# vitoplantamura/OnnxStream

Hardware: NVIDIA H100
Metric: SD1.5 UNet 512x512 bs=1 denoise steps/s (one UNet Model::run per step) (higher is better)
Workload: dtype f16

## Files before the change

### include/onnxstream_b200_kernels.h

```cpp
#ifndef ONNXSTREAM_B200_KERNELS_H
#define ONNXSTREAM_B200_KERNELS_H

#include <stddef.h>
#include <stdint.h>

#ifdef __cplusplus
extern "C" {
#endif

enum { OSB_NONE = 0, OSB_U8 = 1, OSB_F16 = 2, OSB_F32 = 3, OSB_I64 = 4 };

#define OSB_MAX_DIMS 6

int osb_convert(const void* src, int src_dtype, void* dst, int dst_dtype, size_t n, float scale, int zero_point, void* stream);

enum { OSB_UN_SIGMOID = 0, OSB_UN_SILU, OSB_UN_ERF, OSB_UN_SQRT, OSB_UN_SIN, OSB_UN_COS, OSB_UN_POW, OSB_UN_NEG,
       OSB_UN_GELU_ERF, OSB_UN_COPY, OSB_UN_MULC, OSB_UN_ADDC, OSB_UN_RECIP_SQRT };
int osb_unary(int op, const void* x, void* y, int dtype, size_t n, float alpha, void* stream);

enum { OSB_BIN_ADD = 0, OSB_BIN_SUB, OSB_BIN_MUL, OSB_BIN_DIV, OSB_BIN_MUL_GELU, OSB_BIN_MUL_SIGMOID, OSB_BIN_SILU_MUL  };
int osb_binary(int op, const void* a, const int64_t* a_strides, const void* b, const int64_t* b_strides,
               void* out, const int64_t* out_shape, int ndim, int dtype, void* stream);

int osb_bf16x3_expand_cols(const void* in_f32, void* out_bf16, int64_t rows, int64_t L, int64_t ld_in, int b_side, void* stream);
// ... 7 lines not shown
int osb_tc_gemm_f32x_f16w(const void* A_f32, const void* B_f16, int64_t ldb, void* C_f32, const void* bias_f32, const void* residual_f32, int64_t M, int64_t N,
                          int64_t K, void* planes, void* stream);
int osb_tc_conv_f32x_f16w_ok(int64_t H, int64_t W, int64_t Cin, int64_t Cout, int kh, int kw, int stride, int64_t Ho, int64_t Wo);
int osb_tc_conv_f32x_f16w(const void* x_f32, const void* w_f16, const void* bias_f32, const void* residual_f32, void* y_f32, int64_t H, int64_t W, int64_t Cin,
                          int64_t Cout, int kh, int kw, int stride, int pad_top, int pad_left, int64_t Ho, int64_t Wo, void* planes, void* stream);
int osb_concat2(const void* a, const void* b, void* out, int64_t outer, int64_t a_bytes, int64_t b_bytes, void* stream);
int osb_strided_copy(const void* in, void* out, int elem_size, int ndim, const int64_t* shape,
                     const int64_t* in_stride, const int64_t* in_div, int64_t in_offset,
                     const int64_t* out_stride, int64_t out_offset, void* stream);

int osb_transpose2d(const void* in, void* out, int elem_size, int64_t batch, int64_t rows, int64_t cols, void* stream);

int osb_softmax(const void* x, void* y, int dtype, int64_t rows, int64_t cols, void* stream);

int osb_softmax_scaled(const void* x, void* y, int dtype, int64_t rows, int64_t cols, float scale, const void* mask, int64_t mask_rows, void* stream);
int osb_softmax_scaled_ld(const void* x, void* y, int dtype, int64_t rows, int64_t cols, int64_t ld, float scale, const void* mask, int64_t mask_rows, void* stream);

int osb_instance_norm(const void* x, void* y, int dtype, int64_t channels, int64_t n_per_channel,
                      const void* scale, const void* bias, float eps, void* stream);

int osb_group_norm(const void* x, void* y, int dtype, int nhwc, int64_t C, int64_t HW, int groups,
                   const void* gamma, const void* beta, float eps, int fuse_silu, void* stats, void* stream);

int osb_geglu(const void* x, void* y, int dtype, int64_t rows, int64_t inner, void* stream);
int osb_tc_gemm_geglu(const void* A, const void* B, void* y, const void* bias, int64_t M, int64_t inner, int64_t K, void* stream);

int osb_layer_norm(const void* x, void* y, int dtype, int64_t rows, int64_t cols, const void* gamma, const void* beta,
                   float eps, void* stream);

int osb_reduce_mean(const void* x, void* y, int dtype, int64_t rows, int64_t cols, void* stream);

int osb_gather_rows(const void* table, const int64_t* idx, void* out, int64_t n_idx, int64_t table_rows, int64_t row_bytes, void* stream);

int osb_gemm(const void* A, const void* B, void* C, const void* bias, const void* residual,
             int64_t batch, int64_t M, int64_t N, int64_t K,
             int64_t stride_a, int64_t stride_b, int64_t stride_c, int b_transposed, int dtype, int impl, void* stream);

int osb_gemm_grouped(const void* A, const void* const* B, void* const* C, int groups, int64_t M, int64_t N, int64_t K,
                     int b_transposed, int dtype, int impl, void* stream);

int osb_gemm_ld(const void* A, int64_t lda, const void* B, int64_t ldb, void* C, int64_t ldc, const void* bias, const void* residual,
                int64_t batch, int64_t M, int64_t N, int64_t K, int64_t stride_a, int64_t stride_b, int64_t stride_c,
                int b_transposed, int dtype, int impl, void* stream);

int osb_conv2d(const void* x, const void* w, const void* bias, const void* residual, void* y,
               int64_t H, int64_t W, int64_t Cin, int64_t Cout, int kh, int kw, int stride, int pad_top, int pad_left,
               int64_t Ho, int64_t Wo, int dtype, int impl, void* stream);
int osb_conv2d_ex(const void* x, const void* w, const void* bias, const void* bias2, const void* residual, void* y, int64_t H, int64_t W, int64_t Cin, int64_t Cout,
                  int kh, int kw, int stride, int pad_top, int pad_left, int64_t Ho, int64_t Wo, int dtype, int impl, void* stream,
                  void* gn_stats, int gn_groups, int* gn_done);
int osb_conv2d_fusable(const void* x, const void* w, const void* y, int64_t H, int64_t W, int64_t Cin, int64_t Cout, int kh, int kw, int stride, int dtype, int impl);
int osb_rms_norm(const void* x, int xd, const void* w, int wd, void* y, int yd, int64_t rows, int64_t cols, float eps, void* stream);
int osb_rope(const void* x, const void* cs, const void* sn, void* y, int dtype, int64_t rows, int64_t D, int64_t table_rows, void* stream);
int osb_gemv_w8(const void* A, const void* Wq, void* C, const void* bias, const void* residual, int64_t M, int64_t N, int64_t K, float wscale, int wzp, int dtype, void* stream);
int osb_gemv_f16w(const void* A, const void* W, int64_t ldb, void* C, const void* bias, const void* residual, int64_t M, int64_t N, int64_t K, void* stream);
int osb_gemv_grouped(const void* A, const void* const* B, void* const* C, const int64_t* N, const float* wscale, const int* wzp, int groups,
                     int64_t M, int64_t K, int wdtype, int dtype, void* stream);
int osb_qu8_tc_gemm_ok(int64_t M, int64_t N, int64_t K, const void* A, const void* B, const void* C);
int osb_qu8_tc_conv_ok(int64_t Cin, int64_t Cout, int64_t Ho, int64_t Wo, int kh, int kw, int stride, const void* x, const void* w, const void* y);
int osb_rowsum_u8(const void* x, void* out, int64_t rows, int64_t cols, void* stream);
int osb_colsum_u8(const void* w, void* out, int64_t K, int64_t N, void* stream);
int osb_pad_sum_u8(const void* x, void* xp, void* psum, int64_t H, int64_t W, int64_t C, int64_t Hp, int64_t Wp, int pad_top, int pad_left, int zx, void* stream);
int osb_qu8_tc_gemm(const void* A, const void* B, void* C, const void* bias, const void* rsum, const void* csum, int64_t M, int64_t N, int64_t K, int bt,
                    int zx, float sx, int zw, float sw, int zy, float sy, void* stream);
int osb_qu8_tc_conv(const void* xp, const void* psum, const void* w, const void* bias, const void* csum, void* y, int64_t Hp, int64_t Wp, int64_t Cin, int64_t Cout,
                    int kh, int kw, int stride, int64_t Ho, int64_t Wo, int zx, float sx, int zw, float sw, int zy, float sy, void* stream);
int osb_binary_qu8(int op, const void* a, const int64_t* as, float sa, int za, const void* b, const int64_t* bs, float sb, int zb,
                   void* out, float so, int zo, const int64_t* shape, int ndim, void* stream);
int osb_softmax_qu8(const void* x, void* y, int64_t rows, int64_t cols, float in_scale, float out_scale, int out_zp, void* stream);
int osb_percentiles(const void* x, int dtype, size_t n, int threads, float from_left, float from_right, void* out3, void* stream);
float osb_percentile_key_to_float(unsigned key, int dtype);
int osb_channel_add_stats(const void* x, const void* addv, void* y, int dtype, int64_t C, int64_t HW, int groups, void* stats, void* stream);
int osb_concat2_stats(const void* a, const void* b, void* y, int dtype, int64_t ca, int64_t cb, int64_t HW, int groups, void* stats, void* stream);
int osb_group_norm_apply(const void* x, void* y, int dtype, int64_t C, int64_t HW, int groups, const void* gamma, const void* beta, float eps, int fuse_silu,
                         const void* stats, void* clear_stats, void* stream);

int osb_attention(const void* q, const void* k, const void* v, const void* mask, void* out,
                  int64_t heads, int64_t Tq, int64_t Tk, int64_t d, int64_t dv, float scale, int k_transposed,
                  int64_t kv_group, int dtype, void* stream);

int osb_flash_attention_ok(int64_t T, int64_t Tk, int64_t d, int dtype);
int osb_flash_attention(const void* q, int64_t ldq, const void* k, int64_t ldk, const void* v, int64_t ldv, void* out, int64_t ldo,
                        int64_t heads, int64_t T, int64_t Tk, int64_t d, float scale, void* stream);

int osb_flash_attention_f32x_ok(int64_t T, int64_t Tk, int64_t d, int dtype);
int osb_flash_attention_f32x(const void* q, int64_t ldq, const void* k, int64_t ldk, const void* v, int64_t ldv, void* out, int64_t ldo,
                             int64_t heads, int64_t T, int64_t Tk, int64_t d, float scale, void* planes, void* stream);

int osb_flash_attention_wide_ok(int64_t T, int64_t Tk, int64_t d, int dtype);
int osb_flash_attention_wide(const void* q, const void* k, const void* v, void* out, int64_t heads, int64_t T, int64_t Tk, int64_t d,
                             float scale, int k_transposed, int dtype, void* stream);

int osb_flash_attention_wide_f32x_ok(int64_t T, int64_t Tk, int64_t d, int dtype);
int osb_flash_attention_wide_f32x(const void* q, const void* k, const void* v, void* out, int64_t heads, int64_t T, int64_t Tk, int64_t d,
                                  float scale, int k_transposed, void* planes, void* stream);

int osb_sdpa_flash_ok(int64_t Hq, int64_t Hkv, int64_t Tq, int64_t Tk, int64_t d, int64_t dv, int dtype);
int osb_sdpa_flash(const void* q, const void* k, const void* v, const void* mask, void* out,
                   int64_t Hq, int64_t Hkv, int64_t Tq, int64_t Tk, int64_t d, float scale, void* stream);

int osb_sdpa_flash_f32x_ok(int64_t Hq, int64_t Hkv, int64_t Tq, int64_t Tk, int64_t d, int64_t dv, int dtype);
int osb_sdpa_flash_f32x(const void* q, const void* k, const void* v, const void* mask, void* out,
                        int64_t Hq, int64_t Hkv, int64_t Tq, int64_t Tk, int64_t d, float scale,
                        void* planes, void* stream);

int osb_gemm_qu8(const uint8_t* A, const uint8_t* B, uint8_t* C, const int32_t* bias, int64_t M, int64_t N, int64_t K,
                 int zx, float sx, int zw, float sw, int zy, float sy, void* stream);
int osb_conv2d_qu8(const uint8_t* x, const uint8_t* w, const int32_t* bias, uint8_t* y,
                   int64_t H, int64_t W, int64_t Cin, int64_t Cout, int kh, int kw, int stride, int pad_top, int pad_left,
                   int64_t Ho, int64_t Wo, int zx, float sx, int zw, float sw, int zy, float sy, void* stream);

int osb_scatter_elems(void* out, const int64_t* pos, const void* updates, int64_t n, int elem_size, void* stream);

int osb_maxpool_nhwc(const void* x, void* y, int dtype, int64_t H, int64_t W, int64_t C, int kh, int kw, int stride, int pad_top,
                     int pad_left, int64_t Ho, int64_t Wo, void* stream);

int osb_fill(void* dst, int dtype, size_t n, float value, void* stream);

int osb_gemm_tc_eligible(int64_t M, int64_t N, int64_t K, int dtype);

void osb_tc_set_pair_mode(int mode);

void osb_tc_set_tile(int bm, int bn, int split);

void osb_tc_profile(int enable);
int osb_tc_profile_read(double* out4);
int osb_tc_profile_dump(char* buf, int cap);

int osb_pdl_enabled(void);
void osb_set_pdl(int enable);

uint64_t osb_launch_count(void);
void osb_launch_count_reset(void);
uint64_t osb_tc_launch_count(void);

#ifdef __cplusplus
}
#endif
#endif
```

### onnxstream_b200/csrc/attention_wgmma.cu

```cuda

#include "common.cuh"
#include "tc_ptx.cuh"
#include <cuda.h>
#include <cstdio>

namespace {

using namespace tcptx;

constexpr int BQ = 128;
constexpr int BKV = 128;
constexpr int KV_STAGES = 4;
constexpr int FA_THREADS = 384;
constexpr int FA_CONSUMERS = 256;
constexpr int FA_PRODUCER_REGS = 40, FA_CONSUMER_REGS = 232;

template <int NCH, int BK, int QKS, int KS = KV_STAGES, int PLANES = 1>
struct FaCfg {
    static_assert(QKS <= 4 * NCH && (BK == 32 || BK == 64 || BK == 128), "tile");
    static constexpr int Q_CHUNK = BQ * 128;
    static constexpr int KV_CHUNK = BK * 128;
    static constexpr int Q_PLANE = NCH * Q_CHUNK;
    static constexpr int KV_PLANE = NCH * KV_CHUNK;
    static constexpr int Q_BYTES = PLANES * Q_PLANE;
    static constexpr int KV_BYTES = PLANES * KV_PLANE;
    static constexpr int BARS = Q_BYTES + KS * 2 * KV_BYTES;
    static constexpr int SMEM = BARS + 1024 + 256;
};

struct FaParams {
    int T, Tk, d;
    int kv_tiles;
    float scale_log2;
    __half* out;
    long long ldo;
};

__device__ __forceinline__ uint8_t* fa_prologue(const CUtensorMap* map_q, const CUtensorMap* map_k, const CUtensorMap* map_v, int bar_off,
                                                uint32_t arrivals, int n0, int n1 = 0)
{
    extern __shared__ uint8_t smem_raw[];
    uint8_t* smem = (uint8_t*)(((uintptr_t)smem_raw + 1023) & ~(uintptr_t)1023);
    const int warp = threadIdx.x >> 5, lane = threadIdx.x & 31;
    if (warp == 0 && lane == 0) {
        asm volatile("prefetch.tensormap [%0];" ::"l"(map_q) : "memory");
        asm volatile("prefetch.tensormap [%0];" ::"l"(map_k) : "memory");
        asm volatile("prefetch.tensormap [%0];" ::"l"(map_v) : "memory");
    }
    if (warp == 1 && lane == 0) {
        uint64_t* bars = (uint64_t*)(smem + bar_off);
        mbar_init(bars, 1);
        for (int i = 0; i < n0; i++) { mbar_init(&bars[1 + i], 1); mbar_init(&bars[1 + n0 + i], arrivals); }
        for (int i = 0; i < n1; i++) { mbar_init(&bars[1 + 2 * n0 + i], 1); mbar_init(&bars[1 + 2 * n0 + n1 + i], arrivals); }
        asm volatile("fence.mbarrier_init.release.cluster;" ::: "memory");
    }
    __syncthreads();
    osb_pdl_wait();
    return smem;
}

template <int KS, typename Load>
__device__ __forceinline__ void fa_produce_kv(uint64_t* kv_full, uint64_t* kv_empty, int n_kv, uint32_t tile_bytes, Load load)
{
    for (int j = 0; j < n_kv; j++) {
        const int st = j % KS;
        mbar_wait(&kv_empty[st], ((j / KS) & 1) ^ 1);
        if (elect_one()) {
            mbar_expect_tx(&kv_full[st], tile_bytes);
            load(st, j, &kv_full[st]);
        }
        __syncwarp();
    }
    osb_pdl_trigger_late();
}

template <int BK>
__device__ __forceinline__ float fa_row_max(const float (&s)[BK / 2], int h)
{
    float mt = -INFINITY;
#pragma unroll
    for (int c = 0; c < BK / 8; c++) mt = fmaxf(mt, fmaxf(s[4 * c + 2 * h], s[4 * c + 2 * h + 1]));
    mt = fmaxf(mt, __shfl_xor_sync(0xffffffffu, mt, 1));
    mt = fmaxf(mt, __shfl_xor_sync(0xffffffffu, mt, 2));
    return mt;
}

__device__ __forceinline__ float ex2_approx(float x)
{
    float y;
    asm("ex2.approx.ftz.f32 %0, %1;" : "=f"(y) : "f"(x));
    return y;
}

__device__ __forceinline__ uint32_t pack_half2(float lo, float hi)
{
    __half2 h2 = __floats2half2_rn(lo, hi);
    return *reinterpret_cast<uint32_t*>(&h2);
}

__device__ __forceinline__ void store_pair(__half* p, float lo, float hi) { *reinterpret_cast<uint32_t*>(p) = pack_half2(lo, hi); }
__device__ __forceinline__ void store_pair(float* p, float lo, float hi) { *reinterpret_cast<float2*>(p) = make_float2(lo, hi); }

template <typename OutT, int NCH>
__device__ __forceinline__ void fa_store(const float (&o)[NCH][32], const float (&l_run)[2], OutT* const (&rows)[2], int ncols, int cq)
{
#pragma unroll
    for (int h = 0; h < 2; h++) {
        float l = l_run[h];
        l += __shfl_xor_sync(0xffffffffu, l, 1);
        l += __shfl_xor_sync(0xffffffffu, l, 2);
        const float inv = 1.f / l;
        if (!rows[h]) continue;
#pragma unroll
        for (int ch = 0; ch < NCH; ch++)
#pragma unroll
            for (int c = 0; c < 8; c++) {
                const int col = 64 * ch + 8 * c + cq;
                if (col < ncols) store_pair(rows[h] + col, o[ch][4 * c + 2 * h] * inv, o[ch][4 * c + 2 * h + 1] * inv);
            }
    }
}

template <int BK>
__device__ __forceinline__ void qk_mma(float (&s)[BK / 2], uint64_t da, uint64_t db, uint32_t scale_d = 1u)
{
    if constexpr (BK == 128) wgmma_m64n128k16_f16<0>(s, da, db, scale_d);
    else if constexpr (BK == 64) wgmma_m64n64k16_f16<0>(s, da, db, scale_d);
    else wgmma_m64n32k16_f16<0>(s, da, db, scale_d);
}

template <int NCH, int BK, int QKS>
__device__ __forceinline__ void fa_issue_qk(float (&s)[BK / 2], uint64_t qdesc, uint64_t kdesc)
{
    using C = FaCfg<NCH, BK, QKS>;
    fence_regs(s);
    wgmma_fence();
#pragma unroll
    for (int k = 0; k < QKS; k++)
        qk_mma<BK>(s, qdesc + (uint64_t)(((k >> 2) * C::Q_CHUNK >> 4) + (k & 3) * 2), kdesc + (uint64_t)(((k >> 2) * C::KV_CHUNK >> 4) + (k & 3) * 2), k > 0);
    wgmma_commit();
}

template <int NCH, int BK, int QKS>
__device__ __forceinline__ void fa_issue_pv(float (&o)[NCH][32], uint32_t (&a)[BK / 16][4], uint64_t vdesc)
{
    using C = FaCfg<NCH, BK, QKS>;
#pragma unroll
    for (int ch = 0; ch < NCH; ch++) fence_regs(o[ch]);
    fence_regs(a);
    wgmma_fence();
#pragma unroll
    for (int kk = 0; kk < BK / 16; kk++)
#pragma unroll
        for (int ch = 0; ch < NCH; ch++)
            wgmma_m64n64k16_f16_rs(o[ch], a[kk], vdesc + (uint64_t)((ch * C::KV_CHUNK + kk * 2048) >> 4), 1u);
    wgmma_commit();
}

template <int BK>
__device__ __forceinline__ void fa_softmax(float (&s)[BK / 2], float (&m_run)[2], float (&l_run)[2], float (&alpha)[2], int key0, int cq, const FaParams& p)
{
    if (key0 + BK > p.Tk) {
#pragma unroll
        for (int c = 0; c < BK / 8; c++)
#pragma unroll
            for (int e = 0; e < 2; e++)
                if (key0 + 8 * c + cq + e >= p.Tk) { s[4 * c + e] = -INFINITY; s[4 * c + 2 + e] = -INFINITY; }
    }
    float neg_m[2];
#pragma unroll
    for (int h = 0; h < 2; h++) {
        const float m_new = fmaxf(m_run[h], fa_row_max<BK>(s, h) * p.scale_log2);
        alpha[h] = ex2_approx(m_run[h] - m_new);
        neg_m[h] = -m_new;
        m_run[h] = m_new;
    }
    float lsum[2] = { 0.f, 0.f };
#pragma unroll
    for (int c = 0; c < BK / 8; c++)
#pragma unroll
        for (int h = 0; h < 2; h++)
#pragma unroll
            for (int e = 0; e < 2; e++) {
                const float pe = ex2_approx(fmaf(s[4 * c + 2 * h + e], p.scale_log2, neg_m[h]));
                s[4 * c + 2 * h + e] = pe;
                lsum[h] += pe;
            }
#pragma unroll
    for (int h = 0; h < 2; h++) l_run[h] = l_run[h] * alpha[h] + lsum[h];
}

template <int NCH, int BK>
__device__ __forceinline__ void fa_rescale_pack(float (&o)[NCH][32], uint32_t (&a)[BK / 16][4], const float (&s)[BK / 2], const float (&alpha)[2])
{
#pragma unroll
    for (int ch = 0; ch < NCH; ch++)
#pragma unroll
        for (int c = 0; c < 8; c++)
#pragma unroll
            for (int h = 0; h < 2; h++) { o[ch][4 * c + 2 * h] *= alpha[h]; o[ch][4 * c + 2 * h + 1] *= alpha[h]; }
#pragma unroll
    for (int c = 0; c < BK / 8; c++)
#pragma unroll
        for (int h = 0; h < 2; h++) a[c >> 1][(c & 1) * 2 + h] = pack_half2(s[4 * c + 2 * h], s[4 * c + 2 * h + 1]);
}

template <int NCH, int BK, int QKS>
__global__ void __launch_bounds__(FA_THREADS, 1)
flash_attention_kernel(const __grid_constant__ CUtensorMap map_q, const __grid_constant__ CUtensorMap map_k, const __grid_constant__ CUtensorMap map_v,
                       const FaParams p)
{
    using C = FaCfg<NCH, BK, QKS>;
    constexpr int S = KV_STAGES;
    osb_pdl_trigger_entry();
    const int warp = threadIdx.x >> 5, lane = threadIdx.x & 31;
    const int head = blockIdx.y;
    const int q0 = blockIdx.x * BQ;
    const int n_kv = p.kv_tiles;
    uint8_t* smem = fa_prologue(&map_q, &map_k, &map_v, C::BARS, FA_CONSUMERS / 32, S);
    uint8_t* sQ = smem;
    uint8_t* sK = sQ + C::Q_BYTES;
    uint8_t* sV = sK + S * C::KV_BYTES;
    uint64_t* q_full = (uint64_t*)(smem + C::BARS);
    uint64_t* kv_full = q_full + 1;
    uint64_t* kv_empty = kv_full + S;

    if (warp < 4) {
        setmaxnreg_dec<FA_PRODUCER_REGS>();
        if (warp == 0) {
            if (elect_one()) {
                mbar_expect_tx(q_full, C::Q_BYTES);
#pragma unroll
                for (int c = 0; c < NCH; c++) tma_load_3d(sQ + c * C::Q_CHUNK, &map_q, q_full, 64 * c, head, q0);
            }
            __syncwarp();
            fa_produce_kv<S>(kv_full, kv_empty, n_kv, 2 * C::KV_BYTES, [&](int st, int j, uint64_t* bar) {
#pragma unroll
                for (int c = 0; c < NCH; c++) {
                    tma_load_3d(sK + st * C::KV_BYTES + c * C::KV_CHUNK, &map_k, bar, 64 * c, head, j * BK);
                    tma_load_3d(sV + st * C::KV_BYTES + c * C::KV_CHUNK, &map_v, bar, 64 * c, head, j * BK);
                }
            });
        }
    } else {
        setmaxnreg_inc<FA_CONSUMER_REGS>();
        const int wg = (warp >> 2) - 1;
        const int r = (warp & 3) * 16 + (lane >> 2);
        const int cq = 2 * (lane & 3);
        const uint32_t my_bar = 1 + wg, other_bar = 2 - wg;
        if (wg == 0) named_bar_arrive(my_bar, FA_CONSUMERS);
        const uint64_t qdesc = make_smem_desc(smem_u32(sQ) + wg * (BQ / 2) * 128, 16, 1024);
        const uint64_t kdesc0 = make_smem_desc(smem_u32(sK), 16, 1024);
        const uint64_t vdesc0 = make_smem_desc(smem_u32(sV), C::KV_CHUNK, 1024);
        float o[NCH][32];
#pragma unroll
        for (int ch = 0; ch < NCH; ch++)
#pragma unroll
            for (int i = 0; i < 32; i++) o[ch][i] = 0.f;
        float s[BK / 2];
        uint32_t a[BK / 16][4];
        float m_run[2] = { -INFINITY, -INFINITY }, l_run[2] = { 0.f, 0.f }, alpha[2];
        mbar_wait(q_full, 0);

        mbar_wait(&kv_full[0], 0);
        named_bar_sync(my_bar, FA_CONSUMERS);
        fa_issue_qk<NCH, BK, QKS>(s, qdesc, kdesc0);
        named_bar_arrive(other_bar, FA_CONSUMERS);
        wgmma_wait<0>();
        fence_regs(s);
        fa_softmax<BK>(s, m_run, l_run, alpha, 0, cq, p);
        fa_rescale_pack<NCH, BK>(o, a, s, alpha);
        for (int j = 1; j < n_kv; j++) {
            const int st = j % S, prev = (j - 1) % S;
            mbar_wait(&kv_full[st], (j / S) & 1);
            named_bar_sync(my_bar, FA_CONSUMERS);
            fa_issue_qk<NCH, BK, QKS>(s, qdesc, kdesc0 + (uint64_t)(st * C::KV_BYTES >> 4));
            fa_issue_pv<NCH, BK, QKS>(o, a, vdesc0 + (uint64_t)(prev * C::KV_BYTES >> 4));
            named_bar_arrive(other_bar, FA_CONSUMERS);
            wgmma_wait<1>();
            fence_regs(s);
            fa_softmax<BK>(s, m_run, l_run, alpha, j * BK, cq, p);
            wgmma_wait<0>();
#pragma unroll
            for (int ch = 0; ch < NCH; ch++) fence_regs(o[ch]);
            fence_regs(a);
            __syncwarp();
            if (lane == 0) mbar_arrive(&kv_empty[prev]);
            fa_rescale_pack<NCH, BK>(o, a, s, alpha);
        }
        named_bar_sync(my_bar, FA_CONSUMERS);
        fa_issue_pv<NCH, BK, QKS>(o, a, vdesc0 + (uint64_t)((n_kv - 1) % S * C::KV_BYTES >> 4));
        if (wg == 0) named_bar_arrive(other_bar, FA_CONSUMERS);
        wgmma_wait<0>();
#pragma unroll
        for (int ch = 0; ch < NCH; ch++) fence_regs(o[ch]);
        __half* rows[2];
#pragma unroll
        for (int h = 0; h < 2; h++) {
            const int qrow = q0 + wg * (BQ / 2) + r + 8 * h;
            rows[h] = qrow < p.T ? p.out + (long long)qrow * p.ldo + (long long)head * p.d : nullptr;
        }
        fa_store(o, l_run, rows, p.d, cq);
    }
}

template <auto Kernel, typename... Args>
int fa_launch_kernel(dim3 grid, int threads, int smem, cudaStream_t st, const Args&... args)
{
    static bool attr = false;
    if (!attr) {
        cudaError_t e = cudaFuncSetAttribute(Kernel, cudaFuncAttributeMaxDynamicSharedMemorySize, smem);
        if (e != cudaSuccess) return (int)e;
        attr = true;
    }
    osb_launch(Kernel, grid, threads, (size_t)smem, st, args...);
    return launched(1);
}

struct SdpaParams {
    int rows;
    int Tq, Tk, d;
    int kv_tiles;
    float scale_log2;
    const __half* mask;
    __half* out;
};

__device__ __forceinline__ uint32_t ld_mask_pair(const __half* row, int col, int Tk, bool vec)
{
    const unsigned short* m = reinterpret_cast<const unsigned short*>(row) + col;
    if (col + 1 < Tk) {
        if (vec) return __ldg(reinterpret_cast<const unsigned int*>(m));
        return (uint32_t)__ldg(m) | ((uint32_t)__ldg(m + 1) << 16);
    }
    return col < Tk ? (uint32_t)__ldg(m) : 0u;
}

template <int NCH, int BK>
__global__ void __launch_bounds__(FA_THREADS, 1)
sdpa_flash_kernel(const __grid_constant__ CUtensorMap map_q, const __grid_constant__ CUtensorMap map_k, const __grid_constant__ CUtensorMap map_v,
                  const SdpaParams p)
{
    using C = FaCfg<NCH, BK, 4 * NCH>;
    constexpr float LOG2E = 1.4426950408889634f;
    osb_pdl_trigger_entry();
    const int warp = threadIdx.x >> 5, lane = threadIdx.x & 31;
    const int r0 = blockIdx.x * BQ, hk = blockIdx.y;
    const int n_kv = p.kv_tiles;
    uint8_t* smem = fa_prologue(&map_q, &map_k, &map_v, C::BARS, FA_CONSUMERS, KV_STAGES);
    uint8_t* sQ = smem;
    uint8_t* sK = sQ + C::Q_BYTES;
    uint8_t* sV = sK + KV_STAGES * C::KV_BYTES;
    uint64_t* q_full = (uint64_t*)(smem + C::BARS);
    uint64_t* kv_full = q_full + 1;
    uint64_t* kv_empty = kv_full + KV_STAGES;

    if (warp == 0) {
        if (elect_one()) {
            mbar_expect_tx(q_full, C::Q_BYTES);
#pragma unroll
            for (int c = 0; c < NCH; c++) tma_load_3d(sQ + c * C::Q_CHUNK, &map_q, q_full, 64 * c, r0, hk);
        }
        __syncwarp();
        fa_produce_kv<KV_STAGES>(kv_full, kv_empty, n_kv, 2 * C::KV_BYTES, [&](int st, int j, uint64_t* bar) {
#pragma unroll
            for (int c = 0; c < NCH; c++) {
                tma_load_3d(sK + st * C::KV_BYTES + c * C::KV_CHUNK, &map_k, bar, 64 * c, j * BK, hk);
                tma_load_3d(sV + st * C::KV_BYTES + c * C::KV_CHUNK, &map_v, bar, 64 * c, j * BK, hk);
            }
        });
    } else if (warp >= 4) {
        const int wg = (warp >> 2) - 1;
        const int r = (warp & 3) * 16 + (lane >> 2);
        const int cq = 2 * (lane & 3);
        const uint64_t qdesc = make_smem_desc(smem_u32(sQ) + wg * (BQ / 2) * 128, 16, 1024);
        const uint64_t kdesc0 = make_smem_desc(smem_u32(sK), 16, 1024);
        const uint64_t vdesc0 = make_smem_desc(smem_u32(sV), C::KV_CHUNK, 1024);
        const bool has_mask = p.mask != nullptr, vec = (p.Tk & 1) == 0;
        const __half* mrow[2];
#pragma unroll
        for (int h = 0; h < 2; h++) {
            const int R = r0 + wg * (BQ / 2) + r + 8 * h;
// ... 5 lines not shown
#pragma unroll
            for (int i = 0; i < 32; i++) o[ch][i] = 0.f;
        float m_run[2] = { -INFINITY, -INFINITY }, l_run[2] = { 0.f, 0.f };
        mbar_wait(q_full, 0);
        for (int j = 0; j < n_kv; j++) {
            const int ks = j % KV_STAGES;
            const int key0 = j * BK;
            mbar_wait(&kv_full[ks], (j / KV_STAGES) & 1);
            float s[BK / 2];
            fa_issue_qk<NCH, BK, 4 * NCH>(s, qdesc, kdesc0 + (uint64_t)(ks * C::KV_BYTES >> 4));
            uint32_t mk[2][BK / 8];
#pragma unroll
            for (int h = 0; h < 2; h++)
#pragma unroll
                for (int c = 0; c < BK / 8; c++) mk[h][c] = has_mask ? ld_mask_pair(mrow[h], key0 + 8 * c + cq, p.Tk, vec) : 0u;
            wgmma_wait<0>();
            const bool tail = key0 + BK > p.Tk;
#pragma unroll
            for (int c = 0; c < BK / 8; c++)
#pragma unroll
                for (int h = 0; h < 2; h++) {
                    __half2 m2 = *reinterpret_cast<__half2*>(&mk[h][c]);
                    const float2 mf = __half22float2(m2);
                    float x0 = fmaf(s[4 * c + 2 * h], p.scale_log2, mf.x * LOG2E);
                    float x1 = fmaf(s[4 * c + 2 * h + 1], p.scale_log2, mf.y * LOG2E);
                    if (tail) {
                        if (key0 + 8 * c + cq >= p.Tk) x0 = -INFINITY;
                        if (key0 + 8 * c + cq + 1 >= p.Tk) x1 = -INFINITY;
                    }
                    s[4 * c + 2 * h] = x0; s[4 * c + 2 * h + 1] = x1;
                }
            float alpha[2], neg_m[2];
#pragma unroll
            for (int h = 0; h < 2; h++) {
                const float m_new = fmaxf(m_run[h], fa_row_max<BK>(s, h));
                const bool none = m_new == -INFINITY;
                alpha[h] = none ? 1.f : ex2_approx(m_run[h] - m_new);
                neg_m[h] = none ? 0.f : -m_new;
                m_run[h] = m_new;
            }
            float lsum[2] = { 0.f, 0.f };
#pragma unroll
            for (int c = 0; c < BK / 8; c++) {
#pragma unroll
                for (int h = 0; h < 2; h++) {
                    const float p0 = ex2_approx(s[4 * c + 2 * h] + neg_m[h]);
                    const float p1 = ex2_approx(s[4 * c + 2 * h + 1] + neg_m[h]);
                    lsum[h] += p0 + p1;
                    s[4 * c + 2 * h] = p0; s[4 * c + 2 * h + 1] = p1;
                }
            }
#pragma unroll
            for (int h = 0; h < 2; h++) l_run[h] = l_run[h] * alpha[h] + lsum[h];
            uint32_t a[BK / 16][4];
            fa_rescale_pack<NCH, BK>(o, a, s, alpha);
            fa_issue_pv<NCH, BK, 4 * NCH>(o, a, vdesc0 + (uint64_t)(ks * C::KV_BYTES >> 4));
            wgmma_wait<0>();
            mbar_arrive(&kv_empty[ks]);
        }
        __half* rows[2];
#pragma unroll
        for (int h = 0; h < 2; h++) {
            const int R = r0 + wg * (BQ / 2) + r + 8 * h;
            rows[h] = R < p.rows ? p.out + ((long long)hk * p.rows + R) * p.d : nullptr;
        }
        fa_store(o, l_run, rows, p.d, cq);
    }
}

template <int NCH, int BK>
int sdpa_launch(const void* q, const void* k, const void* v, SdpaParams p, int64_t Hkv, cudaStream_t st)
{
    using C = FaCfg<NCH, BK, 4 * NCH>;
    const uint64_t d = p.d;
    CUtensorMap mq, mk, mv;
    if (!make_map(&mq, q, d, p.rows, Hkv, d * 2, p.rows * d * 2, 64, BQ, 1) || !make_map(&mk, k, d, p.Tk, Hkv, d * 2, p.Tk * d * 2, 64, BK, 1) ||
        !make_map(&mv, v, d, p.Tk, Hkv, d * 2, p.Tk * d * 2, 64, BK, 1))
        return (int)cudaErrorInvalidValue;
    p.kv_tiles = (p.Tk + BK - 1) / BK;
    dim3 grid((unsigned)((p.rows + BQ - 1) / BQ), (unsigned)Hkv);
    return fa_launch_kernel<sdpa_flash_kernel<NCH, BK>>(grid, FA_THREADS, C::SMEM, st, mq, mk, mv, p);
}

template <int NCH, int BK, int QKS>
int fa_launch(const void* q, int64_t ldq, const void* k, int64_t ldk, const void* v, int64_t ldv, FaParams p, int64_t heads, cudaStream_t st)
{
    using C = FaCfg<NCH, BK, QKS>;
    const uint64_t d = p.d;
    CUtensorMap mq, mk, mv;
    if (!make_map(&mq, q, d, heads, p.T, d * 2, ldq * 2, 64, 1, BQ) || !make_map(&mk, k, d, heads, p.Tk, d * 2, ldk * 2, 64, 1, BK) ||
        !make_map(&mv, v, d, heads, p.Tk, d * 2, ldv * 2, 64, 1, BK))
        return (int)cudaErrorInvalidValue;
    p.kv_tiles = (p.Tk + BK - 1) / BK;
    dim3 grid((unsigned)((p.T + BQ - 1) / BQ), (unsigned)heads);
    return fa_launch_kernel<flash_attention_kernel<NCH, BK, QKS>>(grid, FA_THREADS, C::SMEM, st, mq, mk, mv, p);
}

constexpr int WD_BQ = 64;
constexpr int WD_BK = 64;
constexpr int WD_NV = 4;
constexpr int WD_DCH = 8;
constexpr int WD_K_STAGES = 8, WD_V_STAGES = 2;
constexpr int WD_THREADS = 256, WD_CONSUMERS = 128;
constexpr int WD_PRODUCER_REGS = 40, WD_CONSUMER_REGS = 240;
constexpr int WD_Q_CHUNK = WD_BQ * 128;
constexpr int WD_K_CHUNK = WD_BK * 128;
constexpr int WD_V_CHUNK = WD_BK * 128;
constexpr int WD_V_BYTES = WD_NV * WD_V_CHUNK;
constexpr int WD_BARS = WD_DCH * WD_Q_CHUNK + WD_K_STAGES * WD_K_CHUNK + WD_V_STAGES * WD_V_BYTES;
constexpr int WD_SMEM = WD_BARS + 1024 + 256;

template <bool KT>
__device__ __forceinline__ void wd_issue_qk_chunk(float (&s)[WD_BK / 2], uint64_t qdesc, uint64_t kdesc, bool first)
{
#pragma unroll
    for (int k = 0; k < 4; k++)
        wgmma_m64n64k16_f16<KT ? 1 : 0>(s, qdesc + (uint64_t)(k * 2), kdesc + (uint64_t)(KT ? (k * 2048) >> 4 : k * 2), (first && k == 0) ? 0u : 1u);
    wgmma_commit();
}

__device__ __forceinline__ void wd_issue_pv(float (&o)[WD_NV][32], uint32_t (&a)[WD_BK / 16][4], uint64_t vdesc)
{
#pragma unroll
    for (int ch = 0; ch < WD_NV; ch++) fence_regs(o[ch]);
    fence_regs(a);
    wgmma_fence();
#pragma unroll
    for (int kk = 0; kk < WD_BK / 16; kk++)
#pragma unroll
        for (int ch = 0; ch < WD_NV; ch++)
            wgmma_m64n64k16_f16_rs(o[ch], a[kk], vdesc + (uint64_t)((ch * WD_V_CHUNK + kk * 2048) >> 4), 1u);
    wgmma_commit();
}

template <bool KT>
__global__ void __launch_bounds__(WD_THREADS, 1)
flash_attention_wide_kernel(const __grid_constant__ CUtensorMap map_q, const __grid_constant__ CUtensorMap map_k,
                            const __grid_constant__ CUtensorMap map_v, const FaParams p)
{
    constexpr int KS = WD_K_STAGES, VS = WD_V_STAGES;
    osb_pdl_trigger_entry();
    const int warp = threadIdx.x >> 5, lane = threadIdx.x & 31;
    const int n_slices = (p.d + 64 * WD_NV - 1) / (64 * WD_NV);
    const int col0 = (blockIdx.x % n_slices) * (64 * WD_NV);
    const int q0 = (blockIdx.x / n_slices) * WD_BQ;
    const int head = blockIdx.y;
    const int n_dch = (p.d + 63) >> 6;
    uint8_t* smem = fa_prologue(&map_q, &map_k, &map_v, WD_BARS, WD_CONSUMERS / 32, KS, VS);
    uint8_t* sQ = smem;
    uint8_t* sK = sQ + WD_DCH * WD_Q_CHUNK;
    uint8_t* sV = sK + KS * WD_K_CHUNK;
    uint64_t* q_full = (uint64_t*)(smem + WD_BARS);
    uint64_t* k_full = q_full + 1;
    uint64_t* k_empty = k_full + KS;
    uint64_t* v_full = k_empty + KS;
    uint64_t* v_empty = v_full + VS;
    const int n_kv = p.kv_tiles;

    if (warp < 4) {
        setmaxnreg_dec<WD_PRODUCER_REGS>();
        if (warp == 0) {
            if (elect_one()) {
                mbar_expect_tx(q_full, n_dch * WD_Q_CHUNK);
                for (int c = 0; c < n_dch; c++) tma_load_3d(sQ + c * WD_Q_CHUNK, &map_q, q_full, 64 * c, q0, head);
            }
            __syncwarp();
            const int n_vch = min(WD_NV, (p.d - col0 + 63) >> 6);
            int kc = 0;
            for (int j = 0; j < n_kv; j++) {
                for (int c = 0; c < n_dch; c++, kc++) {
                    const int st = kc % KS;
                    mbar_wait(&k_empty[st], ((kc / KS) & 1) ^ 1);
                    if (elect_one()) {
                        mbar_expect_tx(&k_full[st], WD_K_CHUNK);
                        if (KT) tma_load_3d(sK + st * WD_K_CHUNK, &map_k, &k_full[st], j * WD_BK, 64 * c, head);
                        else tma_load_3d(sK + st * WD_K_CHUNK, &map_k, &k_full[st], 64 * c, j * WD_BK, head);
                    }
                    __syncwarp();
// ... 668 lines not shown
                for (int h = 0; h < 2; h++) {
                    __nv_bfloat16 p0[3], p1[3];
                    bf16x3_split(s[4 * c + 2 * h], p0[0], p0[1], p0[2]);
                    bf16x3_split(s[4 * c + 2 * h + 1], p1[0], p1[1], p1[2]);
#pragma unroll
                    for (int pl = 0; pl < 3; pl++) a[pl][c >> 1][(c & 1) * 2 + h] = pack_bf162(p0[pl], p1[pl]);
                }
#pragma unroll
            for (int pl = 0; pl < 3; pl++) fence_regs(a[pl]);
#pragma unroll
            for (int ch = 0; ch < NCH; ch++) {
                float t[32];
                fence_regs(t);
                wgmma_fence();
#pragma unroll
                for (int xx = 0; xx < 6; xx++)
#pragma unroll
                    for (int kk = 0; kk < BK / 16; kk++) {
                        const int x = 5 - xx;
                        wgmma_m64n64k16_bf16_rs(t, a[x3a(x)][kk], vdesc + (uint64_t)((x3b(x) * C::KV_PLANE + ch * C::KV_CHUNK + kk * 2048) >> 4), (kk | xx) != 0);
                    }
                wgmma_commit();
                wgmma_wait<0>();
                fence_regs(t);
#pragma unroll
                for (int i = 0; i < 32; i++) o[ch][i] += t[i];
            }
#pragma unroll
            for (int pl = 0; pl < 3; pl++) fence_regs(a[pl]);
            __syncwarp();
            if (lane == 0) mbar_arrive(&kv_empty[st]);
        }
        float* rows[2];
#pragma unroll
        for (int h = 0; h < 2; h++) {
            const int R = r0 + wg * (BQ / 2) + r + 8 * h;
            rows[h] = R < p.rows ? p.out + ((long long)hk * p.rows + R) * p.d : nullptr;
        }
        fa_store(o, l_run, rows, p.d, cq);
    }
}

template <int NCH, int BK, int QKS, int KS>
int sdpa_f32x_launch(const float* q, const float* k, const float* v, SdpaF32xParams p, int64_t Hkv, __nv_bfloat16* planes, cudaStream_t st)
{
    using Cf = FaCfg<NCH, BK, QKS, KS, 3>;
    const int64_t rows = p.rows, Tk = p.Tk, d = p.d;
    __nv_bfloat16* pq = planes;
    __nv_bfloat16* pk = pq + 3 * Hkv * rows * d;
    __nv_bfloat16* pv = pk + 3 * Hkv * Tk * d;
    CUtensorMap mq, mk, mv;
    if (!make_map(&mq, pq, 3 * d, rows, Hkv, 3 * d * 2, rows * 3 * d * 2, 64, BQ, 1) ||
        !make_map(&mk, pk, d, Tk, 3 * Hkv, d * 2, Tk * d * 2, 64, BK, 1) ||
        !make_map(&mv, pv, 3 * d, Tk, Hkv, 3 * d * 2, Tk * 3 * d * 2, 64, BK, 1))
        return (int)cudaErrorInvalidValue;
    osb_launch((f32x_split_kernel), grid_for((size_t)(Hkv * rows * d / 4), 256), 256, 0, st, q, d, q, d, q, d, pq, pq, pq, Hkv * rows,
               (int64_t)0, (int)d);
    int e = launched();
    if (e) return e;
    osb_launch((f32x_split_kernel), grid_for((size_t)(Hkv * Tk * d / 4), 256), 256, 0, st, v, d, v, d, v, d, pv, pv, pv, Hkv * Tk,
               (int64_t)0, (int)d);
    if ((e = launched())) return e;
    const dim3 kgrid((unsigned)((Tk + 31) / 32), (unsigned)((d + 31) / 32), (unsigned)Hkv), kblock(32, 8);
    osb_launch((f32x_split_k_kernel<false>), kgrid, kblock, 0, st, k, pk, (int)Tk, (int)d);
    if ((e = launched())) return e;
    p.kv_tiles = (int)((Tk + BK - 1) / BK);
    dim3 grid((unsigned)((rows + BQ - 1) / BQ), (unsigned)Hkv);
    return fa_launch_kernel<sdpa_flash_f32x_kernel<NCH, BK, QKS, KS>>(grid, FA_THREADS, Cf::SMEM, st, mq, mk, mv, p);
}

}

int osb_f32x_split_rows(const float* x, __nv_bfloat16* planes, int64_t rows, int64_t C, cudaStream_t st)
{
    osb_launch((f32x_split_kernel), grid_for((size_t)(rows * C / 4), 256), 256, 0, st, x, C, x, C, x, C, planes, planes, planes, rows, (int64_t)0, (int)C);
    return launched();
}

extern "C" int osb_flash_attention_ok(int64_t T, int64_t Tk, int64_t d, int dtype)
{
    return dtype == OSB_F16 && T >= 64 && fa_dims_ok(T, Tk, d) && get_encode() != nullptr;
}

extern "C" int osb_flash_attention(const void* q, int64_t ldq, const void* k, int64_t ldk, const void* v, int64_t ldv, void* out, int64_t ldo,
                                   int64_t heads, int64_t T, int64_t Tk, int64_t d, float scale, void* stream)
{
    if (heads * T == 0) return 0;
    if (!fa_dims_ok(T, Tk, d) || !fa_launch_ok(heads, scale) || (ldq % 8) || (ldk % 8) || (ldv % 8) || (ldo % 8) || !aligned16(q, k, v, out))
        return (int)cudaErrorInvalidValue;
    FaParams p{};
    p.T = (int)T; p.Tk = (int)Tk; p.d = (int)d;
    p.scale_log2 = scale * 1.4426950408889634f;
    p.out = (__half*)out; p.ldo = ldo;
    cudaStream_t st = (cudaStream_t)stream;
    if (d <= 48) return fa_launch<1, 128, 3>(q, ldq, k, ldk, v, ldv, p, heads, st);
    if (d <= 64) return fa_launch<1, 128, 4>(q, ldq, k, ldk, v, ldv, p, heads, st);
    if (d <= 80) return fa_launch<2, 64, 5>(q, ldq, k, ldk, v, ldv, p, heads, st);
    if (d <= 128) return fa_launch<2, 64, 8>(q, ldq, k, ldk, v, ldv, p, heads, st);
    return fa_launch<3, 32, 10>(q, ldq, k, ldk, v, ldv, p, heads, st);
}

extern "C" int osb_flash_attention_f32x_ok(int64_t T, int64_t Tk, int64_t d, int dtype)
{
    return dtype == OSB_F32 && fa_dims_ok(T, Tk, d) && get_encode() != nullptr;
}

extern "C" int osb_flash_attention_f32x(const void* q, int64_t ldq, const void* k, int64_t ldk, const void* v, int64_t ldv, void* out, int64_t ldo,
                                        int64_t heads, int64_t T, int64_t Tk, int64_t d, float scale, void* planes, void* stream)
{
    if (!osb_flash_attention_f32x_ok(T, Tk, d, OSB_F32) || !fa_launch_ok(heads, scale)) return (int)cudaErrorInvalidValue;
    const int64_t C = heads * d;
    if (ldq < C || ldk < C || ldv < C || ldo < C || (ldq % 4) || (ldk % 4) || (ldv % 4) || (ldo % 4) || C > INT32_MAX) return (int)cudaErrorInvalidValue;
    if (!aligned16(q, k, v, out, planes)) return (int)cudaErrorInvalidValue;
    FaParams p{};
    p.T = (int)T; p.Tk = (int)Tk; p.d = (int)d;
    p.out = nullptr; p.ldo = ldo;
    const float* fq = (const float*)q; const float* fk = (const float*)k; const float* fv = (const float*)v;
    float* fo = (float*)out;
    __nv_bfloat16* pl = (__nv_bfloat16*)planes;
    cudaStream_t st = (cudaStream_t)stream;
    if (d <= 48) return f32x_launch<1, 64, 3, 2>(fq, ldq, fk, ldk, fv, ldv, fo, p, scale, heads, pl, st);
    if (d <= 64) return f32x_launch<1, 64, 4, 2>(fq, ldq, fk, ldk, fv, ldv, fo, p, scale, heads, pl, st);
    if (d <= 80) return f32x_launch<2, 32, 5, 2>(fq, ldq, fk, ldk, fv, ldv, fo, p, scale, heads, pl, st);
    if (d <= 128) return f32x_launch<2, 32, 8, 2>(fq, ldq, fk, ldk, fv, ldv, fo, p, scale, heads, pl, st);
    return f32x_launch<3, 32, 10, 1>(fq, ldq, fk, ldk, fv, ldv, fo, p, scale, heads, pl, st);
}

extern "C" int osb_flash_attention_wide_ok(int64_t T, int64_t Tk, int64_t d, int dtype)
{
    return dtype == OSB_F16 && d > 160 && d <= 64 * WD_DCH && d % 8 == 0 && T >= 1 && Tk >= 1 && T <= (int64_t)INT32_MAX - WD_BQ &&
           Tk <= (int64_t)INT32_MAX - WD_BK && get_encode() != nullptr;
}

extern "C" int osb_flash_attention_wide(const void* q, const void* k, const void* v, void* out, int64_t heads, int64_t T, int64_t Tk, int64_t d,
                                        float scale, int k_transposed, int dtype, void* stream)
{
    if (!osb_flash_attention_wide_ok(T, Tk, d, dtype) || !fa_launch_ok(heads, scale) || (k_transposed && Tk % 8) || !aligned16(q, k, v, out))
        return (int)cudaErrorInvalidValue;
    FaParams p{};
    p.T = (int)T; p.Tk = (int)Tk; p.d = (int)d;
    p.scale_log2 = scale * 1.4426950408889634f;
    p.out = (__half*)out; p.ldo = d;
    cudaStream_t st = (cudaStream_t)stream;
    return k_transposed ? wd_launch<true>(q, k, v, p, heads, st) : wd_launch<false>(q, k, v, p, heads, st);
}

extern "C" int osb_flash_attention_wide_f32x_ok(int64_t T, int64_t Tk, int64_t d, int dtype)
{
    return dtype == OSB_F32 && d > 160 && d <= 64 * WD_DCH && d % 8 == 0 && T >= 1 && Tk >= 1 && T <= (int64_t)INT32_MAX - WD_BQ &&
           Tk <= (int64_t)INT32_MAX - WX_BK && get_encode() != nullptr;
}

extern "C" int osb_flash_attention_wide_f32x(const void* q, const void* k, const void* v, void* out, int64_t heads, int64_t T, int64_t Tk,
                                             int64_t d, float scale, int k_transposed, void* planes, void* stream)
{
    if (!osb_flash_attention_wide_f32x_ok(T, Tk, d, OSB_F32) || !fa_launch_ok(heads, scale) || !aligned16(q, k, v, out, planes))
        return (int)cudaErrorInvalidValue;
    FaParams p{};
    p.T = (int)T; p.Tk = (int)Tk; p.d = (int)d;
    p.out = nullptr; p.ldo = d;
    return wx_launch((const float*)q, (const float*)k, (const float*)v, (float*)out, p, scale, heads, k_transposed != 0, (__nv_bfloat16*)planes,
                     (cudaStream_t)stream);
}

extern "C" int osb_sdpa_flash_ok(int64_t Hq, int64_t Hkv, int64_t Tq, int64_t Tk, int64_t d, int64_t dv, int dtype)
{
    return dtype == OSB_F16 && d == dv && d >= 8 && d <= 128 && d % 8 == 0 && Hkv >= 1 && Hkv <= 65535 && Hq >= Hkv && Hq % Hkv == 0 &&
           Tq >= 1 && Tk >= 1 && (Hq / Hkv) * Tq <= (int64_t)INT32_MAX - BQ && Tk <= (int64_t)INT32_MAX - BKV && get_encode() != nullptr;
}

extern "C" int osb_sdpa_flash(const void* q, const void* k, const void* v, const void* mask, void* out,
                              int64_t Hq, int64_t Hkv, int64_t Tq, int64_t Tk, int64_t d, float scale, void* stream)
{
    if (Hq * Tq * d == 0) return 0;
    if (!osb_sdpa_flash_ok(Hq, Hkv, Tq, Tk, d, d, OSB_F16)) return (int)cudaErrorInvalidValue;
    if (!aligned16(q, k, v, out) || ((uintptr_t)mask & 3) != 0) return (int)cudaErrorInvalidValue;
    SdpaParams p{};
    p.rows = (int)((Hq / Hkv) * Tq); p.Tq = (int)Tq; p.Tk = (int)Tk; p.d = (int)d;
    p.scale_log2 = scale * 1.4426950408889634f;
    p.mask = (const __half*)mask; p.out = (__half*)out;
    cudaStream_t st = (cudaStream_t)stream;
    return d <= 64 ? sdpa_launch<1, 128>(q, k, v, p, Hkv, st) : sdpa_launch<2, 64>(q, k, v, p, Hkv, st);
// ... 28 lines not shown
```

Measured before the change: 197.9.

## Generalize flash attention to variable consumer warpgroups and pick query tile by wave cost

```diff
diff --git a/include/onnxstream_b200_kernels.h b/include/onnxstream_b200_kernels.h
--- a/include/onnxstream_b200_kernels.h
+++ b/include/onnxstream_b200_kernels.h
@@ -113,6 +113,8 @@
 int osb_flash_attention_ok(int64_t T, int64_t Tk, int64_t d, int dtype);
 int osb_flash_attention(const void* q, int64_t ldq, const void* k, int64_t ldk, const void* v, int64_t ldv, void* out, int64_t ldo,
                         int64_t heads, int64_t T, int64_t Tk, int64_t d, float scale, void* stream);
+int osb_flash_attention_tiles(const void* q, int64_t ldq, const void* k, int64_t ldk, const void* v, int64_t ldv, void* out, int64_t ldo,
+                              int64_t heads, int64_t T, int64_t Tk, int64_t d, float scale, int rows, int per_sm, void* stream);
 
 int osb_flash_attention_f32x_ok(int64_t T, int64_t Tk, int64_t d, int dtype);
 int osb_flash_attention_f32x(const void* q, int64_t ldq, const void* k, int64_t ldk, const void* v, int64_t ldv, void* out, int64_t ldo,
diff --git a/onnxstream_b200/csrc/attention_wgmma.cu b/onnxstream_b200/csrc/attention_wgmma.cu
--- a/onnxstream_b200/csrc/attention_wgmma.cu
+++ b/onnxstream_b200/csrc/attention_wgmma.cu
@@ -15,10 +15,10 @@
 constexpr int FA_CONSUMERS = 256;
 constexpr int FA_PRODUCER_REGS = 40, FA_CONSUMER_REGS = 232;
 
-template <int NCH, int BK, int QKS, int KS = KV_STAGES, int PLANES = 1>
+template <int NCH, int BK, int QKS, int KS = KV_STAGES, int PLANES = 1, int QROWS = BQ>
 struct FaCfg {
     static_assert(QKS <= 4 * NCH && (BK == 32 || BK == 64 || BK == 128), "tile");
-    static constexpr int Q_CHUNK = BQ * 128;
+    static constexpr int Q_CHUNK = QROWS * 128;
     static constexpr int KV_CHUNK = BK * 128;
     static constexpr int Q_PLANE = NCH * Q_CHUNK;
     static constexpr int KV_PLANE = NCH * KV_CHUNK;
@@ -129,10 +129,10 @@
     else wgmma_m64n32k16_f16<0>(s, da, db, scale_d);
 }
 
-template <int NCH, int BK, int QKS>
+template <int NCH, int BK, int QKS, int QROWS = BQ>
 __device__ __forceinline__ void fa_issue_qk(float (&s)[BK / 2], uint64_t qdesc, uint64_t kdesc)
 {
-    using C = FaCfg<NCH, BK, QKS>;
+    using C = FaCfg<NCH, BK, QKS, KV_STAGES, 1, QROWS>;
     fence_regs(s);
     wgmma_fence();
 #pragma unroll
@@ -205,19 +205,32 @@
         for (int h = 0; h < 2; h++) a[c >> 1][(c & 1) * 2 + h] = pack_half2(s[4 * c + 2 * h], s[4 * c + 2 * h + 1]);
 }
 
-template <int NCH, int BK, int QKS>
-__global__ void __launch_bounds__(FA_THREADS, 1)
+template <int NWG, int MINB>
+struct FaShape {
+    static_assert(NWG >= 1 && NWG <= 4 && MINB >= 1, "shape");
+    static constexpr int ROWS = 64 * NWG;
+    static constexpr int THREADS = 128 * (NWG + 1);
+    static constexpr int CONSUMERS = 128 * NWG;
+    static constexpr int REGS = (65536 / (THREADS * MINB)) & ~7;
+    static constexpr int PRODUCER_REGS = (NWG <= 2 && MINB == 1) ? FA_PRODUCER_REGS : 24;
+    static constexpr int CONSUMER_REGS_FIT = (((NWG + 1) * (REGS < 256 ? REGS : 256) - PRODUCER_REGS) / NWG) & ~7;
+    static constexpr int CONSUMER_REGS = CONSUMER_REGS_FIT < FA_CONSUMER_REGS ? CONSUMER_REGS_FIT : FA_CONSUMER_REGS;
+};
+
+template <int NCH, int BK, int QKS, int NWG = 2, int MINB = 1>
+__global__ void __launch_bounds__(FaShape<NWG, MINB>::THREADS, MINB)
 flash_attention_kernel(const __grid_constant__ CUtensorMap map_q, const __grid_constant__ CUtensorMap map_k, const __grid_constant__ CUtensorMap map_v,
                        const FaParams p)
 {
-    using C = FaCfg<NCH, BK, QKS>;
+    using Sh = FaShape<NWG, MINB>;
+    using C = FaCfg<NCH, BK, QKS, KV_STAGES, 1, Sh::ROWS>;
     constexpr int S = KV_STAGES;
     osb_pdl_trigger_entry();
     const int warp = threadIdx.x >> 5, lane = threadIdx.x & 31;
     const int head = blockIdx.y;
-    const int q0 = blockIdx.x * BQ;
+    const int q0 = blockIdx.x * Sh::ROWS;
     const int n_kv = p.kv_tiles;
-    uint8_t* smem = fa_prologue(&map_q, &map_k, &map_v, C::BARS, FA_CONSUMERS / 32, S);
+    uint8_t* smem = fa_prologue(&map_q, &map_k, &map_v, C::BARS, Sh::CONSUMERS / 32, S);
     uint8_t* sQ = smem;
     uint8_t* sK = sQ + C::Q_BYTES;
     uint8_t* sV = sK + S * C::KV_BYTES;
@@ -226,7 +239,7 @@
     uint64_t* kv_empty = kv_full + S;
 
     if (warp < 4) {
-        setmaxnreg_dec<FA_PRODUCER_REGS>();
+        setmaxnreg_dec<Sh::PRODUCER_REGS>();
         if (warp == 0) {
             if (elect_one()) {
                 mbar_expect_tx(q_full, C::Q_BYTES);
@@ -243,13 +256,14 @@
             });
         }
     } else {
-        setmaxnreg_inc<FA_CONSUMER_REGS>();
+        setmaxnreg_inc<Sh::CONSUMER_REGS>();
         const int wg = (warp >> 2) - 1;
         const int r = (warp & 3) * 16 + (lane >> 2);
         const int cq = 2 * (lane & 3);
-        const uint32_t my_bar = 1 + wg, other_bar = 2 - wg;
-        if (wg == 0) named_bar_arrive(my_bar, FA_CONSUMERS);
-        const uint64_t qdesc = make_smem_desc(smem_u32(sQ) + wg * (BQ / 2) * 128, 16, 1024);
+        constexpr bool turns = NWG > 1;
+        const uint32_t my_bar = 1 + wg, other_bar = NWG == 2 ? 2 - wg : (wg == NWG - 1 ? 1 : 2 + wg);
+        if (turns && wg == 0) named_bar_arrive(my_bar, 256);
+        const uint64_t qdesc = make_smem_desc(smem_u32(sQ) + wg * 64 * 128, 16, 1024);
         const uint64_t kdesc0 = make_smem_desc(smem_u32(sK), 16, 1024);
         const uint64_t vdesc0 = make_smem_desc(smem_u32(sV), C::KV_CHUNK, 1024);
         float o[NCH][32];
@@ -263,9 +277,9 @@
         mbar_wait(q_full, 0);
 
         mbar_wait(&kv_full[0], 0);
-        named_bar_sync(my_bar, FA_CONSUMERS);
-        fa_issue_qk<NCH, BK, QKS>(s, qdesc, kdesc0);
-        named_bar_arrive(other_bar, FA_CONSUMERS);
+        if (turns) named_bar_sync(my_bar, 256);
+        fa_issue_qk<NCH, BK, QKS, Sh::ROWS>(s, qdesc, kdesc0);
+        if (turns) named_bar_arrive(other_bar, 256);
         wgmma_wait<0>();
         fence_regs(s);
         fa_softmax<BK>(s, m_run, l_run, alpha, 0, cq, p);
@@ -273,10 +287,10 @@
         for (int j = 1; j < n_kv; j++) {
             const int st = j % S, prev = (j - 1) % S;
             mbar_wait(&kv_full[st], (j / S) & 1);
-            named_bar_sync(my_bar, FA_CONSUMERS);
-            fa_issue_qk<NCH, BK, QKS>(s, qdesc, kdesc0 + (uint64_t)(st * C::KV_BYTES >> 4));
+            if (turns) named_bar_sync(my_bar, 256);
+            fa_issue_qk<NCH, BK, QKS, Sh::ROWS>(s, qdesc, kdesc0 + (uint64_t)(st * C::KV_BYTES >> 4));
             fa_issue_pv<NCH, BK, QKS>(o, a, vdesc0 + (uint64_t)(prev * C::KV_BYTES >> 4));
-            named_bar_arrive(other_bar, FA_CONSUMERS);
+            if (turns) named_bar_arrive(other_bar, 256);
             wgmma_wait<1>();
             fence_regs(s);
             fa_softmax<BK>(s, m_run, l_run, alpha, j * BK, cq, p);
@@ -288,16 +302,16 @@
             if (lane == 0) mbar_arrive(&kv_empty[prev]);
             fa_rescale_pack<NCH, BK>(o, a, s, alpha);
         }
-        named_bar_sync(my_bar, FA_CONSUMERS);
+        if (turns) named_bar_sync(my_bar, 256);
         fa_issue_pv<NCH, BK, QKS>(o, a, vdesc0 + (uint64_t)((n_kv - 1) % S * C::KV_BYTES >> 4));
-        if (wg == 0) named_bar_arrive(other_bar, FA_CONSUMERS);
+        if (turns && (NWG == 2 ? wg == 0 : wg != NWG - 1)) named_bar_arrive(other_bar, 256);
         wgmma_wait<0>();
 #pragma unroll
         for (int ch = 0; ch < NCH; ch++) fence_regs(o[ch]);
         __half* rows[2];
 #pragma unroll
         for (int h = 0; h < 2; h++) {
-            const int qrow = q0 + wg * (BQ / 2) + r + 8 * h;
+            const int qrow = q0 + wg * 64 + r + 8 * h;
             rows[h] = qrow < p.T ? p.out + (long long)qrow * p.ldo + (long long)head * p.d : nullptr;
         }
         fa_store(o, l_run, rows, p.d, cq);
@@ -469,18 +483,20 @@
     return fa_launch_kernel<sdpa_flash_kernel<NCH, BK>>(grid, FA_THREADS, C::SMEM, st, mq, mk, mv, p);
 }
 
-template <int NCH, int BK, int QKS>
+template <int NCH, int BK, int QKS, int NWG = 2, int MINB = 1>
 int fa_launch(const void* q, int64_t ldq, const void* k, int64_t ldk, const void* v, int64_t ldv, FaParams p, int64_t heads, cudaStream_t st)
 {
-    using C = FaCfg<NCH, BK, QKS>;
+    using Sh = FaShape<NWG, MINB>;
+    using C = FaCfg<NCH, BK, QKS, KV_STAGES, 1, Sh::ROWS>;
+    static_assert(MINB * (C::SMEM + 1024) <= 228 * 1024, "shared memory per SM");
     const uint64_t d = p.d;
     CUtensorMap mq, mk, mv;
-    if (!make_map(&mq, q, d, heads, p.T, d * 2, ldq * 2, 64, 1, BQ) || !make_map(&mk, k, d, heads, p.Tk, d * 2, ldk * 2, 64, 1, BK) ||
+    if (!make_map(&mq, q, d, heads, p.T, d * 2, ldq * 2, 64, 1, Sh::ROWS) || !make_map(&mk, k, d, heads, p.Tk, d * 2, ldk * 2, 64, 1, BK) ||
         !make_map(&mv, v, d, heads, p.Tk, d * 2, ldv * 2, 64, 1, BK))
         return (int)cudaErrorInvalidValue;
     p.kv_tiles = (p.Tk + BK - 1) / BK;
-    dim3 grid((unsigned)((p.T + BQ - 1) / BQ), (unsigned)heads);
-    return fa_launch_kernel<flash_attention_kernel<NCH, BK, QKS>>(grid, FA_THREADS, C::SMEM, st, mq, mk, mv, p);
+    dim3 grid((unsigned)((p.T + Sh::ROWS - 1) / Sh::ROWS), (unsigned)heads);
+    return fa_launch_kernel<flash_attention_kernel<NCH, BK, QKS, NWG, MINB>>(grid, Sh::THREADS, C::SMEM, st, mq, mk, mv, p);
 }
 
 constexpr int WD_BQ = 64;
@@ -1315,8 +1331,27 @@
     return dtype == OSB_F16 && T >= 64 && fa_dims_ok(T, Tk, d) && get_encode() != nullptr;
 }
 
+static int fa_pick_rows(int64_t T, int64_t heads, int64_t d)
+{
+    static int sms = 0;
+    if (!sms) {
+        int dev = 0;
+        if (cudaGetDevice(&dev) != cudaSuccess || cudaDeviceGetAttribute(&sms, cudaDevAttrMultiProcessorCount, dev) != cudaSuccess || sms < 1) sms = 132;
+    }
+    const int alt = d <= 48 ? 256 : ((d > 64 && d <= 80) || d > 128) ? 64 : 128;
+    auto cost = [&](int64_t rows) { return (heads * ((T + rows - 1) / rows) + sms - 1) / sms * rows; };
+    if (alt > 128) return cost(alt) <= cost(128) ? alt : 128;
+    return cost(alt) < cost(128) ? alt : 128;
+}
+
 extern "C" int osb_flash_attention(const void* q, int64_t ldq, const void* k, int64_t ldk, const void* v, int64_t ldv, void* out, int64_t ldo,
                                    int64_t heads, int64_t T, int64_t Tk, int64_t d, float scale, void* stream)
+{
+    return osb_flash_attention_tiles(q, ldq, k, ldk, v, ldv, out, ldo, heads, T, Tk, d, scale, fa_pick_rows(T, heads, d), 1, stream);
+}
+
+extern "C" int osb_flash_attention_tiles(const void* q, int64_t ldq, const void* k, int64_t ldk, const void* v, int64_t ldv, void* out, int64_t ldo,
+                                         int64_t heads, int64_t T, int64_t Tk, int64_t d, float scale, int rows, int per_sm, void* stream)
 {
     if (heads * T == 0) return 0;
     if (!fa_dims_ok(T, Tk, d) || !fa_launch_ok(heads, scale) || (ldq % 8) || (ldk % 8) || (ldv % 8) || (ldo % 8) || !aligned16(q, k, v, out))
@@ -1326,11 +1361,22 @@
     p.scale_log2 = scale * 1.4426950408889634f;
     p.out = (__half*)out; p.ldo = ldo;
     cudaStream_t st = (cudaStream_t)stream;
-    if (d <= 48) return fa_launch<1, 128, 3>(q, ldq, k, ldk, v, ldv, p, heads, st);
-    if (d <= 64) return fa_launch<1, 128, 4>(q, ldq, k, ldk, v, ldv, p, heads, st);
-    if (d <= 80) return fa_launch<2, 64, 5>(q, ldq, k, ldk, v, ldv, p, heads, st);
-    if (d <= 128) return fa_launch<2, 64, 8>(q, ldq, k, ldk, v, ldv, p, heads, st);
-    return fa_launch<3, 32, 10>(q, ldq, k, ldk, v, ldv, p, heads, st);
+    if (rows == 0) rows = fa_pick_rows(T, heads, d);
+    if (d <= 48) {
+        if (rows == 256 && per_sm == 1) return fa_launch<1, 32, 3, 4, 1>(q, ldq, k, ldk, v, ldv, p, heads, st);
+        if (rows == 128 && per_sm == 1) return fa_launch<1, 128, 3>(q, ldq, k, ldk, v, ldv, p, heads, st);
+        return (int)cudaErrorInvalidValue;
+    }
+    if (d <= 64) return rows == 128 && per_sm == 1 ? fa_launch<1, 128, 4>(q, ldq, k, ldk, v, ldv, p, heads, st) : (int)cudaErrorInvalidValue;
+    if (d <= 80) {
+        if (rows == 64 && per_sm == 1) return fa_launch<2, 64, 5, 1, 1>(q, ldq, k, ldk, v, ldv, p, heads, st);
+        if (rows == 128 && per_sm == 1) return fa_launch<2, 64, 5>(q, ldq, k, ldk, v, ldv, p, heads, st);
+        return (int)cudaErrorInvalidValue;
+    }
+    if (d <= 128) return rows == 128 && per_sm == 1 ? fa_launch<2, 64, 8>(q, ldq, k, ldk, v, ldv, p, heads, st) : (int)cudaErrorInvalidValue;
+    if (rows == 64 && per_sm == 1) return fa_launch<3, 32, 10, 1, 1>(q, ldq, k, ldk, v, ldv, p, heads, st);
+    if (rows == 128 && per_sm == 1) return fa_launch<3, 32, 10>(q, ldq, k, ldk, v, ldv, p, heads, st);
+    return (int)cudaErrorInvalidValue;
 }
 
 extern "C" int osb_flash_attention_f32x_ok(int64_t T, int64_t Tk, int64_t d, int dtype)
```

Result: faster. 201.0 (median of 6 runs) (+1.6%).
